# SDFIdk/malstroem

Hardware: NVIDIA B200
Metric: DEM cells/sec end-to-end (fill->D8->accum->bluespot/watershed labels) (higher is better)
Workload: dtype f32/f64

## Files before the change

malstroem_b200/csrc/common.cuh:

```cuda
#pragma once
#include <cuda_runtime.h>
#include <stdint.h>
#include <stdio.h>

#include "../../include/malstroem_b200.h"

namespace ms {

void set_error(const char *fmt, ...);
extern int64_t g_launches;

#define MS_CUDA(call)                                                                              \
    do {                                                                                           \
        cudaError_t e__ = (call);                                                                  \
        if (e__ != cudaSuccess) {                                                                  \
            ms::set_error("%s:%d: %s -> %s", __FILE__, __LINE__, #call, cudaGetErrorString(e__)); \
            return MS_ERR_CUDA;                                                                    \
        }                                                                                          \
    } while (0)

#define MS_TRY(call)                \
    do {                            \
        int r__ = (call);           \
        if (r__ != MS_OK) return r__; \
    } while (0)

extern int g_prof;
extern int64_t g_prof_units;
void prof_begin(const char *name, cudaStream_t s);
void prof_end(cudaStream_t s);
static inline void prof_units(int64_t u) { g_prof_units = u; }

#define MS_LAUNCH(kernel, grid, block, smem, stream, ...)                                    \
    do {                                                                                     \
        if (ms::g_prof) ms::prof_begin(#kernel, (stream));                                   \
        kernel<<<(grid), (block), (smem), (stream)>>>(__VA_ARGS__);                          \
        if (ms::g_prof) ms::prof_end((stream));                                              \
        ms::g_launches++;                                                                    \
        cudaError_t e__ = cudaGetLastError();                                                \
        if (e__ != cudaSuccess) {                                                            \
            ms::set_error("%s:%d: launch %s -> %s", __FILE__, __LINE__, #kernel,             \
                          cudaGetErrorString(e__));                                          \
            return MS_ERR_CUDA;                                                              \
        }                                                                                    \
    } while (0)

int ensure_init();

extern double g_host_t[4];
int stream_sync(cudaStream_t s);
double now_s();

void *arena_alloc(size_t bytes, cudaStream_t s);
void arena_free(void *p, cudaStream_t s);

template <typename T>
struct DevBuf {
    T *p = nullptr;
    cudaStream_t s = nullptr;
    DevBuf() {}
    DevBuf(const DevBuf &) = delete;
    DevBuf &operator=(const DevBuf &) = delete;
    int alloc(size_t n, cudaStream_t stream) {
        release();
        s = stream;
        if (n == 0) n = 1;
        double t0 = now_s();
        p = (T *)arena_alloc(n * sizeof(T), stream);
        g_host_t[2] += now_s() - t0;
        g_host_t[3] += 1;
        if (!p) {
            set_error("device scratch allocation of %zu bytes failed", n * sizeof(T));
            return MS_ERR_CUDA;
        }
        return MS_OK;
    }
    void release() {
        if (p) arena_free(p, s);
        p = nullptr;
    }
    ~DevBuf() { release(); }
    operator T *() const { return p; }
};

struct HostFlags {
    int64_t *h = nullptr;
    int init();
};
HostFlags &host_flags();
int readback(void *host_pinned, const void *dev, size_t bytes, cudaStream_t s);

static inline unsigned int cdiv(int64_t a, int64_t b) { return (unsigned int)((a + b - 1) / b); }

__host__ __device__ inline uint32_t okey32(float f) {
    f = f + 0.0f;
#ifdef __CUDA_ARCH__
    uint32_t b = __float_as_uint(f);
#else
    union { float f; uint32_t u; } v; v.f = f; uint32_t b = v.u;
#endif
    return (b & 0x80000000u) ? ~b : (b | 0x80000000u);
}
__host__ __device__ inline float okey32_inv(uint32_t k) {
    uint32_t b = (k & 0x80000000u) ? (k & 0x7fffffffu) : ~k;
#ifdef __CUDA_ARCH__
    return __uint_as_float(b);
#else
// ... 146 lines not shown
```

malstroem_b200/csrc/core.cu:

```cuda
#include <stdarg.h>
#include <stdio.h>
#include <stdlib.h>
#include <string.h>

#include <chrono>
#include <algorithm>
#include <map>
#include <string>
#include <vector>

#include "common.cuh"
#include "tma.cuh"

namespace ms {

static thread_local char g_err[1024] = "";
int64_t g_launches = 0;
static int g_device = -1;
static HostFlags g_flags;

void set_error(const char *fmt, ...) {
    va_list ap;
    va_start(ap, fmt);
    vsnprintf(g_err, sizeof(g_err), fmt, ap);
// ... 18 lines not shown

struct ArenaBlock { size_t off, size; bool live; };
static char *g_arena = nullptr;
static size_t g_arena_cap = 0, g_arena_top = 0, g_arena_need = 0, g_overflow_live = 0;
static std::vector<ArenaBlock> g_blocks;
static cudaStream_t g_arena_stream = nullptr;
static std::map<void *, size_t> g_overflow;

void *arena_alloc(size_t bytes, cudaStream_t s) {
    bytes = (bytes + 511) & ~(size_t)511;
    if (s != g_arena_stream) {
        if (g_arena) cudaStreamSynchronize(g_arena_stream);
        g_arena_stream = s;
    }
    if (g_blocks.empty() && g_overflow.empty() && g_arena_need > g_arena_cap) {
        if (g_arena) cudaFree(g_arena);
        g_arena = nullptr;
        size_t want = g_arena_need + (g_arena_need >> 3);
        if (cudaMalloc((void **)&g_arena, want) == cudaSuccess) g_arena_cap = want;
        else { g_arena_cap = 0; cudaGetLastError(); }
        g_arena_top = 0;
    }
    size_t virt = g_arena_top + g_overflow_live + bytes;
    if (virt > g_arena_need) g_arena_need = virt;
    if (g_arena && g_arena_top + bytes <= g_arena_cap) {
        g_blocks.push_back({g_arena_top, bytes, true});
        void *p = g_arena + g_arena_top;
        g_arena_top += bytes;
        return p;
    }
    void *p = nullptr;
    if (cudaMallocAsync(&p, bytes, s) != cudaSuccess) { cudaGetLastError(); return nullptr; }
    g_overflow[p] = bytes;
    g_overflow_live += bytes;
    return p;
}

void arena_free(void *p, cudaStream_t s) {
    auto it = g_overflow.find(p);
    if (it != g_overflow.end()) {
        g_overflow_live -= it->second;
        g_overflow.erase(it);
        cudaFreeAsync(p, s);
        return;
    }
    size_t off = (size_t)((char *)p - g_arena);
    for (size_t k = g_blocks.size(); k-- > 0;)
        if (g_blocks[k].off == off) { g_blocks[k].live = false; break; }
    while (!g_blocks.empty() && !g_blocks.back().live) {
        g_arena_top = g_blocks.back().off;
        g_blocks.pop_back();
    }
}

int g_prof = 0;
int64_t g_prof_units = 0;
struct ProfRec { const char *name; cudaEvent_t a, b; int64_t units; };
static std::vector<ProfRec> g_recs;
static std::vector<cudaEvent_t> g_evpool;

static cudaEvent_t ev_get() {
    if (!g_evpool.empty()) { cudaEvent_t e = g_evpool.back(); g_evpool.pop_back(); return e; }
    cudaEvent_t e;
    cudaEventCreate(&e);
    return e;
}

void prof_begin(const char *name, cudaStream_t s) {
    ProfRec r;
    r.name = name; r.a = ev_get(); r.b = ev_get(); r.units = g_prof_units;
    g_prof_units = 0;
    cudaEventRecord(r.a, s);
    g_recs.push_back(r);
}

void prof_end(cudaStream_t s) { cudaEventRecord(g_recs.back().b, s); }

int HostFlags::init() {
    if (h) return MS_OK;
    MS_CUDA(cudaHostAlloc((void **)&h, 64 * sizeof(int64_t), cudaHostAllocMapped | cudaHostAllocPortable));
    memset(h, 0, 64 * sizeof(int64_t));
    return MS_OK;
}
HostFlags &host_flags() { return g_flags; }

__global__ void k_readback(const uint32_t *__restrict__ src, uint32_t *dst_host, int words) {
    for (int k = threadIdx.x; k < words; k += blockDim.x) dst_host[k] = src[k];
    __threadfence_system();
}

int readback(void *host_pinned, const void *dev, size_t bytes, cudaStream_t s) {
    static int mode = -1;
    if (mode < 0) { const char *e = getenv("MS_READBACK"); mode = (e && e[0] == 'c') ? 0 : 1; }
    if (!mode || (bytes & 3) || bytes > 4096 || ((uintptr_t)dev & 3) || ((uintptr_t)host_pinned & 3)) {
        MS_CUDA(cudaMemcpyAsync(host_pinned, dev, bytes, cudaMemcpyDeviceToHost, s));
        return MS_OK;
    }
    MS_LAUNCH(k_readback, 1, 32, 0, s, (const uint32_t *)dev, (uint32_t *)host_pinned, (int)(bytes >> 2));
    return MS_OK;
}

static int init_device(int device) {
    int n = 0;
    cudaError_t e = cudaGetDeviceCount(&n);
    if (e != cudaSuccess || n == 0) {
        set_error("no CUDA device available (%s): malstroem_b200 has no CPU fallback",
// ... 274 lines not shown
```

malstroem_b200/csrc/fill.cu:

```cuda
#include <string.h>

#include "common.cuh"
#include "tma.cuh"

namespace ms {

constexpr unsigned long long KEY_NONE = ~0ull;

__global__ void __launch_bounds__(256) k_minmax(const float *z, int64_t n, uint32_t *keys, int vec) {
    uint32_t lo = 0xffffffffu, hi = 0u;
    int64_t i = ((int64_t)blockIdx.x * blockDim.x + threadIdx.x) * 4;
    int64_t stride = (int64_t)gridDim.x * blockDim.x * 4;
    for (; i < n; i += stride) {
        if (vec && i + 4 <= n) {
            float4 v = *reinterpret_cast<const float4 *>(z + i);
            uint32_t a = okey32(v.x), b = okey32(v.y), c = okey32(v.z), d = okey32(v.w);
            lo = min(lo, min(min(a, b), min(c, d)));
            hi = max(hi, max(max(a, b), max(c, d)));
        } else {
            for (int64_t j = i; j < n && j < i + 4; j++) {
                uint32_t a = okey32(z[j]);
                lo = min(lo, a);
                hi = max(hi, a);
            }
        }
    }
    lo = __reduce_min_sync(0xffffffffu, lo);
    hi = __reduce_max_sync(0xffffffffu, hi);
    __shared__ uint32_t slo[8], shi[8];
    int lane = threadIdx.x & 31, w = threadIdx.x >> 5;
    if (lane == 0) { slo[w] = lo; shi[w] = hi; }
    __syncthreads();
    if (w == 0) {
        lo = lane < 8 ? slo[lane] : 0xffffffffu;
        hi = lane < 8 ? shi[lane] : 0u;
        lo = __reduce_min_sync(0xffffffffu, lo);
        hi = __reduce_max_sync(0xffffffffu, hi);
        if (lane == 0) {
            atomicMin(&keys[0], lo);
            atomicMax(&keys[1], hi);
        }
    }
}

__global__ void k_minmax_finish(const uint32_t *keys, float *out) {
    out[0] = okey32_inv(keys[0]);
    out[1] = okey32_inv(keys[1]);
}

int minmax_dev(const float *z, int64_t n, float *out2, cudaStream_t s) {
    DevBuf<uint32_t> keys;
    MS_TRY(keys.alloc(2, s));
    static const uint32_t init[2] = {0xffffffffu, 0u};
    MS_CUDA(cudaMemcpyAsync(keys.p, init, sizeof(init), cudaMemcpyHostToDevice, s));
    int64_t want = (n / 4 + 255) / 256;
    int blocks = (int)(want < 1 ? 1 : (want > 148 * 16 ? 148 * 16 : want));
    MS_LAUNCH(k_minmax, blocks, 256, 0, s, z, n, keys.p, (int)(((uintptr_t)z & 15) == 0));
    MS_LAUNCH(k_minmax_finish, 1, 1, 0, s, keys.p, out2);
    return MS_OK;
}
// ... 49 lines not shown
                        if (r + dr < 0 || r + dr >= rows) continue;
                        int j = i + dr * cols + dc;
                        float zj = sz[(lr + 1 + dr) * LD + lc + X0 + dc];
                        if (zj < bz || (zj == bz && j < bi)) { bz = zj; bi = j; bdr = dr; bdc = dc; }
                    }
                int tr = lr + bdr, tc = lc + bdc;
                if (bi == i) t = i;
                else if (tr >= 0 && tr < FT && tc >= 0 && tc < FT) p = (unsigned short)(tr * FT + tc);
                else t = -(1 + bi);
            }
        }
        sp[k] = p;
        tgt[k] = t;
    }
    __syncthreads();
    tile_pointer_double(sp);
    int mine[16], cnt = 0;
#pragma unroll 4
    for (int u = 0; u < 16; u++) {
        int k = tid + 256 * u;
        int lr = k >> 6, lc = k & 63;
        int r = r0 + lr, c = c0 + lc;
        mine[u] = -1;
        if (r < rows && c < cols) {
            int t = tgt[sp[k]];
            int i = r * cols + c;
            if (t < 0) { t = -(t + 1); mine[u] = i; cnt++; }
            ptr[i] = t;
        }
    }
    int pos = block_append_pos(cnt, n_list);
#pragma unroll 4
    for (int u = 0; u < 16; u++)
        if (mine[u] >= 0) list[pos++] = mine[u];
}

__global__ void __launch_bounds__(256) k_catchment_ids(int *ptr_lab, const int *cid, int64_t n) {
    int64_t i = (int64_t)blockIdx.x * blockDim.x + threadIdx.x;
    if (i < n) ptr_lab[i] = cid[ptr_lab[i]];
}

__global__ void __launch_bounds__(256) k_boruvka_init(int *comp, uint32_t *E, int nC) {
    int l = blockIdx.x * blockDim.x + threadIdx.x;
    if (l < nC) {
        comp[l] = l;
        E[l] = okey32(-INFINITY);
    }
}

constexpr unsigned FOREIGN_BIT = 0x80000000u;

constexpr int ME_PER_THREAD = 4;

template <bool FIRST, bool BAND>
__device__ inline bool minedge_cell(const float *__restrict__ z, const int *__restrict__ lab,
                                    const int *__restrict__ comp, const uint8_t *__restrict__ frozen,
                                    unsigned long long *best, int rows, int cols, int i, int r, int c) {
    int l = lab[i];
    int cc = FIRST ? l : (l ? comp[l] : 0);
    if (cc == 0) return false;
    const bool fz = BAND && !FIRST && frozen[cc];
    bool other = false;
    float zc = z[i];
    unsigned long long bk = KEY_NONE;
#pragma unroll
    for (int dr = -1; dr <= 1; dr++)
#pragma unroll
        for (int dc = -1; dc <= 1; dc++) {
            if (dr == 0 && dc == 0) continue;
            int j = i + dr * cols + dc;
            if (r + dr < 0 || r + dr >= rows) {
                if (fz) { other = true; continue; }
                float w = fmaxf(zc, __ldg(z + j));
                if (c < 0) c = i % cols;
                unsigned long long key = ((unsigned long long)okey32(w) << 32) | FOREIGN_BIT | (unsigned)c;
                bk = key < bk ? key : bk;
                continue;
            }
            int lj = __ldg(lab + j);
            if (lj == l) continue;
            if (!FIRST && __ldg(comp + lj) == cc) continue;
            if (fz) { other = true; continue; }
            float w = fmaxf(zc, __ldg(z + j));
            int lo = j < i ? j : i;
            int code = (dr == 0) ? 0 : ((dr * dc == -1) ? 1 : (dc == 0 ? 2 : 3));
            unsigned long long key = ((unsigned long long)okey32(w) << 32) | (unsigned)(((unsigned)lo << 2) | code);
            bk = key < bk ? key : bk;
        }
    if (fz) return other;
    if (bk == KEY_NONE) return false;
    if (bk < best[cc]) atomicMin(&best[cc], bk);
    return true;
}

__device__ __forceinline__ void minedge_append(unsigned keepbits, const int (&cell)[ME_PER_THREAD], int *list_out, int *n_out) {
    __shared__ int wsum[8];
    __shared__ int base_s;
    int cnt = __popc(keepbits), lane = threadIdx.x & 31, w = threadIdx.x >> 5;
    int inc = cnt;
#pragma unroll
    for (int o = 1; o < 32; o <<= 1) {
        int y = __shfl_up_sync(0xffffffffu, inc, o);
        if (lane >= o) inc += y;
    }
    if (lane == 31) wsum[w] = inc;
    __syncthreads();
    if (threadIdx.x == 0) {
        int tot = 0;
        for (int k = 0; k < 8; k++) { int t = wsum[k]; wsum[k] = tot; tot += t; }
        base_s = tot ? atomicAdd(n_out, tot) : 0;
    }
    __syncthreads();
    int pos = base_s + wsum[w] + inc - cnt;
#pragma unroll
    for (int u = 0; u < ME_PER_THREAD; u++)
        if (keepbits & (1u << u)) list_out[pos++] = cell[u];
}

template <bool LIST, bool BAND>
__device__ __forceinline__ void minedge_body(const float *__restrict__ z, const int *__restrict__ lab,
                                                 const int *__restrict__ comp, const uint8_t *__restrict__ frozen,
                                                 unsigned long long *best, int rows, int cols,
                                                 const int *__restrict__ list_in, int n_in, int *list_out, int *n_out) {
    int cell[ME_PER_THREAD];
    unsigned keepbits = 0;
#pragma unroll
    for (int u = 0; u < ME_PER_THREAD; u++) {
        int i = -1, r = 0, c = 0;
        if (LIST) {
            int k = (blockIdx.x * ME_PER_THREAD + u) * 256 + threadIdx.x;
            if (k < n_in) {
                i = list_in[k];
                r = i < cols ? 0 : (i >= (rows - 1) * cols ? rows - 1 : 1);
                c = -1;
            }
        } else {
            c = blockIdx.x * 64 + (threadIdx.x & 63);
            r = (blockIdx.y * ME_PER_THREAD + u) * 4 + (threadIdx.x >> 6);
            if (r < rows && c < cols) i = r * cols + c;
        }
        cell[u] = i;
        if (i >= 0 && minedge_cell<!LIST, BAND>(z, lab, comp, frozen, best, rows, cols, i, r, c)) keepbits |= 1u << u;
    }
    minedge_append(keepbits, cell, list_out, n_out);
}

__global__ void __launch_bounds__(256) k_minedge_first4(const float *__restrict__ z, const int *__restrict__ lab,
                                                        unsigned long long *best, int rows, int cols, int *list_out,
                                                        int *n_out) {
    const int c = (blockIdx.x * 16 + (threadIdx.x & 15)) * 4;
    const int r = blockIdx.y * 16 + (threadIdx.x >> 4);
    int cell[ME_PER_THREAD] = {-1, -1, -1, -1};
    unsigned keepbits = 0;
    if (r > 0 && r < rows - 1 && c < cols) {
        int L[3][6];
        float Z[3][6];
#pragma unroll
        for (int a = 0; a < 3; a++) {
            const size_t row = (size_t)(r - 1 + a) * cols + c;
            const int4 l4 = __ldg(reinterpret_cast<const int4 *>(lab + row));
            const float4 z4 = __ldg(reinterpret_cast<const float4 *>(z + row));
            L[a][1] = l4.x; L[a][2] = l4.y; L[a][3] = l4.z; L[a][4] = l4.w;
            Z[a][1] = z4.x; Z[a][2] = z4.y; Z[a][3] = z4.z; Z[a][4] = z4.w;
            L[a][0] = c > 0 ? __ldg(lab + row - 1) : 0;
            Z[a][0] = c > 0 ? __ldg(z + row - 1) : 0.f;
            L[a][5] = c + 4 < cols ? __ldg(lab + row + 4) : 0;
            Z[a][5] = c + 4 < cols ? __ldg(z + row + 4) : 0.f;
        }
#pragma unroll
        for (int j = 0; j < 4; j++) {
            const int l = L[1][j + 1];
            const int i = r * cols + c + j;
            cell[j] = i;
            if (l == 0) continue;
            const float zc = Z[1][j + 1];
            unsigned long long bk = KEY_NONE;
#pragma unroll
            for (int dr = -1; dr <= 1; dr++)
#pragma unroll
                for (int dc = -1; dc <= 1; dc++) {
                    if (dr == 0 && dc == 0) continue;
                    if (L[1 + dr][j + 1 + dc] == l) continue;
                    const float w = fmaxf(zc, Z[1 + dr][j + 1 + dc]);
                    const int jn = i + dr * cols + dc;
                    const int lo = jn < i ? jn : i;
                    const int code = (dr == 0) ? 0 : ((dr * dc == -1) ? 1 : (dc == 0 ? 2 : 3));
                    const unsigned long long key = ((unsigned long long)okey32(w) << 32) | (unsigned)(((unsigned)lo << 2) | code);
                    bk = key < bk ? key : bk;
                }
            if (bk == KEY_NONE) continue;
            if (bk < best[l]) atomicMin(&best[l], bk);
            keepbits |= 1u << j;
        }
    }
    minedge_append(keepbits, cell, list_out, n_out);
}

template <bool LIST>
__global__ void __launch_bounds__(256) k_minedge(const float *__restrict__ z, const int *__restrict__ lab,
                                                 const int *__restrict__ comp, const uint8_t *__restrict__ frozen,
                                                 unsigned long long *best, int rows, int cols,
                                                 const int *__restrict__ list_in, int n_in, int *list_out, int *n_out) {
    minedge_body<LIST, false>(z, lab, comp, frozen, best, rows, cols, list_in, n_in, list_out, n_out);
}
template <bool LIST>
__global__ void __launch_bounds__(256) k_minedge_band(const float *__restrict__ z, const int *__restrict__ lab,
                                                      const int *__restrict__ comp, const uint8_t *__restrict__ frozen,
                                                      unsigned long long *best, int rows, int cols,
                                                      const int *__restrict__ list_in, int n_in, int *list_out, int *n_out) {
    minedge_body<LIST, true>(z, lab, comp, frozen, best, rows, cols, list_in, n_in, list_out, n_out);
}

__device__ inline int edge_other(int lo, int code, int cols) {
    return lo + (code == 0 ? 1 : (code == 1 ? cols - 1 : (code == 2 ? cols : cols + 1)));
}

__global__ void __launch_bounds__(256) k_hook(const unsigned long long *__restrict__ best,
                                              const int *__restrict__ comp, const int *__restrict__ lab,
                                              int *parent, uint32_t *wk, uint8_t *frozen, int nC, int cols) {
    int k = blockIdx.x * blockDim.x + threadIdx.x;
    if (k >= nC) return;
    parent[k] = k;
    wk[k] = okey32(-INFINITY);
    if (k == 0 || comp[k] != k) return;
    unsigned long long b = best[k];
    if (b == KEY_NONE) return;
    unsigned id = (unsigned)(b & 0xffffffffu);
    if (frozen && (id & FOREIGN_BIT)) {
        frozen[k] = 1;
        return;
    }
    int lo = (int)(id >> 2), code = (int)(id & 3u);
    int hi = edge_other(lo, code, cols);
    int ca = comp[lab[lo]], cb = comp[lab[hi]];
    int t = (ca == k) ? cb : ca;
    wk[k] = (uint32_t)(b >> 32);
    if (t != 0 && best[t] == b && k < t) t = k;
    parent[k] = t;
}

__device__ inline int uf_find(int *parent, int k) {
    int p = parent[k];
    for (;;) {
        int g = parent[p];
        if (g == p) return p;
        parent[k] = g;
        k = p;
        p = g;
    }
}

__global__ void __launch_bounds__(256) k_boruvka_update(int *comp, uint32_t *E, int *parent,
                                                        const uint32_t *__restrict__ wk,
                                                        const uint8_t *__restrict__ frozen, int nC,
                                                        unsigned long long *best, int *remaining) {
    int l = blockIdx.x * blockDim.x + threadIdx.x;
    int live = 0;
    if (l < nC) {
        best[l] = KEY_NONE;
        int k = comp[l];
        if (k != 0) {
            uint32_t e = E[l], w = wk[k];
            if (w > e) E[l] = w;
            int r = uf_find(parent, k);
            comp[l] = r;
            live = (r == l) && !(frozen && frozen[r]);
        }
    }
    int cnt = __syncthreads_count(live);
    if (threadIdx.x == 0 && cnt) atomicAdd(remaining, cnt);
}

__global__ void __launch_bounds__(256) k_fill_final(const float *__restrict__ z, const int *__restrict__ lab,
                                                    const uint32_t *__restrict__ E, float *__restrict__ filled,
                                                    float *__restrict__ depths, int64_t n) {
    int64_t i = (int64_t)blockIdx.x * blockDim.x + threadIdx.x;
    if (i >= n) return;
    float zc = z[i];
    float w = fmaxf(zc, okey32_inv(__ldg(E + lab[i])));
    filled[i] = w;
    if (depths) depths[i] = __fsub_rn(w, zc);
}

static int descent_resolve(const float *dem, int *lab, int *scratch, int64_t rows, int64_t cols, int open,
                           int64_t *rounds_out, cudaStream_t s) {
    DevBuf<int> cnt;
    MS_TRY(cnt.alloc(1, s));
    MS_CUDA(cudaMemsetAsync(cnt.p, 0, sizeof(int), s));
    int tiles_x = (int)cdiv(cols, FT), tiles_y = (int)cdiv(rows, FT);
    prof_units(rows * cols);
    CUtensorMap zmap;
    memset(&zmap, 0, sizeof(zmap));
    if (!open && tma_map_2d(&zmap, dem, rows, cols, FT + 2, DT_LD_TMA, true, true))
        MS_LAUNCH(k_descent_tile<true>, tiles_x * tiles_y, 256, 0, s, dem, lab, (int)rows, (int)cols, tiles_x, open, scratch, cnt.p, zmap);
    else
        MS_LAUNCH(k_descent_tile<false>, tiles_x * tiles_y, 256, 0, s, dem, lab, (int)rows, (int)cols, tiles_x, open, scratch, cnt.p, zmap);
    int64_t *h = host_flags().h;
    MS_TRY(ms::readback(h, cnt.p, sizeof(int), s));
    MS_TRY(ms::stream_sync(s));
    return forest_resolve_list(lab, scratch, *(int *)h, rounds_out, s);
}

static int boruvka_rounds(const float *dem, const int *lab, int *comp, uint32_t *E, uint8_t *frozen, int nC,
                          int64_t rows, int64_t cols, int *rounds_out, const char *what, cudaStream_t s,
                          ms_band *B = nullptr) {
    int64_t n = rows * cols;
    DevBuf<int> parent, counters, listA, listB;
    DevBuf<uint32_t> wk;
    DevBuf<unsigned long long> best;
    MS_TRY(parent.alloc(nC, s));
    MS_TRY(wk.alloc(nC, s));
    MS_TRY(best.alloc(nC, s));
    MS_TRY(counters.alloc(2, s));
    MS_TRY(listA.alloc((size_t)n, s));
    dim3 g2(cdiv(cols, 64), cdiv(rows, 4));
    unsigned gc = cdiv(nC, 256);
    int64_t *h = host_flags().h;
    MS_CUDA(cudaMemsetAsync(best.p, 0xff, (size_t)nC * sizeof(unsigned long long), s));
    int rounds = 0;
    int64_t live = nC - 1;
    int n_list = 0;
    int *lin = nullptr, *lout = listA.p;
    while (live > 0) {
        MS_CUDA(cudaMemsetAsync(counters.p, 0, 2 * sizeof(int), s));
        if (rounds == 0) {
            prof_units(n);
            dim3 g2m(cdiv(cols, 64), cdiv(rows, 4 * ME_PER_THREAD));
            if (frozen)
                MS_LAUNCH(k_minedge_band<false>, g2m, 256, 0, s, dem, lab, (const int *)comp, (const uint8_t *)frozen, best.p,
                          (int)rows, (int)cols, (const int *)nullptr, 0, lout, counters.p + 1);
            else if ((cols & 3) == 0 && ((uintptr_t)dem & 15) == 0 && ((uintptr_t)lab & 15) == 0)
                MS_LAUNCH(k_minedge_first4, dim3(cdiv(cols, 64), cdiv(rows, 16)), 256, 0, s, dem, lab, best.p, (int)rows, (int)cols,
                          lout, counters.p + 1);
            else
                MS_LAUNCH(k_minedge<false>, g2m, 256, 0, s, dem, lab, (const int *)comp, (const uint8_t *)frozen, best.p,
                          (int)rows, (int)cols, (const int *)nullptr, 0, lout, counters.p + 1);
        } else {
            prof_units(n_list);
            if (frozen)
                MS_LAUNCH(k_minedge_band<true>, cdiv(n_list, 256 * ME_PER_THREAD), 256, 0, s, dem, lab, (const int *)comp,
                          (const uint8_t *)frozen, best.p, (int)rows, (int)cols, (const int *)lin, n_list, lout, counters.p + 1);
            else
                MS_LAUNCH(k_minedge<true>, cdiv(n_list, 256 * ME_PER_THREAD), 256, 0, s, dem, lab, (const int *)comp,
                          (const uint8_t *)frozen, best.p, (int)rows, (int)cols, (const int *)lin, n_list, lout, counters.p + 1);
        }
        MS_LAUNCH(k_hook, gc, 256, 0, s, best.p, comp, lab, parent.p, wk.p, frozen, nC, (int)cols);
        MS_LAUNCH(k_boruvka_update, gc, 256, 0, s, comp, E, parent.p, wk.p, (const uint8_t *)frozen, nC, best.p,
                  counters.p);
        MS_TRY(ms::readback(h, counters.p, 2 * sizeof(int), s));
        MS_TRY(ms::stream_sync(s));
        int64_t now = ((int *)h)[0];
        n_list = ((int *)h)[1];
        rounds++;
        if (now >= live || rounds > 64) {
            set_error("%s: Boruvka contraction stalled (%lld -> %lld live components, round %d)", what,
                      (long long)live, (long long)now, rounds);
            return MS_ERR_NOCONV;
        }
        live = now;
        if (live > 0 && n_list == 0) {
            set_error("%s: live components without an outgoing edge", what);
            return MS_ERR_NOCONV;
        }
        if (rounds == 1 && live > 0) MS_TRY(listB.alloc((size_t)n_list, s));
        lin = lout;
        lout = (lout == listA.p) ? listB.p : listA.p;
    }
    if (rounds_out) *rounds_out = rounds;
    if (B) {
        B->n_blist = 0;
        if (rounds > 0 && n_list > 0) {
            int *dst = (int *)band_buf(B, BB_BLIST, (size_t)n_list * sizeof(int));
            if (!dst) return MS_ERR_CUDA;
            MS_CUDA(cudaMemcpyAsync(dst, lin, (size_t)n_list * sizeof(int), cudaMemcpyDeviceToDevice, s));
            MS_TRY(ms::stream_sync(s));
            B->n_blist = n_list;
        }
    }
    return MS_OK;
}

int fill_terrain_dev_impl(const float *dtm, float *filled, float *depths, int64_t rows, int64_t cols,
                          int64_t *stats, cudaStream_t s) {
    if (!dtm || !filled) { set_error("fill_terrain: null pointer"); return MS_ERR_ARG; }
    if (rows < 3 || cols < 3 || rows * cols > (1ll << 30)) {
        set_error("fill_terrain: unsupported shape %lld x %lld", (long long)rows, (long long)cols);
        return MS_ERR_SHAPE;
    }
    int64_t n = rows * cols;
    DevBuf<int> lab, tmp;
    DevBuf<int64_t> total;
    MS_TRY(lab.alloc((size_t)n, s));
    MS_TRY(tmp.alloc((size_t)n, s));
    MS_TRY(total.alloc(1, s));
    dim3 g2(cdiv(cols, 64), cdiv(rows, 4));
    unsigned g1 = cdiv(n, 256);
    int64_t *h = host_flags().h;

    int64_t jump_rounds = 0;
    MS_TRY(descent_resolve(dtm, lab.p, tmp.p, rows, cols, 0, &jump_rounds, s));
    MS_TRY(exclusive_scan_selfptr(lab.p, tmp.p, n, total.p, s));
    MS_LAUNCH(k_catchment_ids, g1, 256, 0, s, lab.p, tmp.p, n);
    MS_TRY(ms::readback(h, total.p, sizeof(int64_t), s));
    MS_TRY(ms::stream_sync(s));
    int nC = (int)h[0];
    tmp.release();

    DevBuf<int> comp;
    DevBuf<uint32_t> E;
    MS_TRY(comp.alloc(nC, s));
    MS_TRY(E.alloc(nC, s));
    MS_LAUNCH(k_boruvka_init, cdiv(nC, 256), 256, 0, s, comp.p, E.p, nC);
    int rounds = 0;
    MS_TRY(boruvka_rounds(dtm, lab.p, comp.p, E.p, nullptr, nC, rows, cols, &rounds, "fill_terrain", s));
    MS_LAUNCH(k_fill_final, g1, 256, 0, s, dtm, lab.p, E.p, filled, depths, n);
    if (stats) { stats[0] = rounds; stats[1] = nC; stats[5] = jump_rounds; }
    return MS_OK;
}


__global__ void __launch_bounds__(256) k_frozen_flags(const int *comp, const uint8_t *frozen, int *flag, int nC) {
    int k = blockIdx.x * blockDim.x + threadIdx.x;
    if (k < nC) flag[k] = (k != 0 && comp[k] == k && frozen[k]) ? 1 : 0;
}

__device__ inline int band_gid(int K, const int *frank, int base) { return K ? 1 + base + frank[K] : 0; }

__global__ void __launch_bounds__(256) k_band_edge_ids(const int *__restrict__ lab, const int *__restrict__ comp,
                                                       const int *__restrict__ frank, int base, int rows, int cols,
                                                       int32_t *top, int32_t *bot) {
    int c = blockIdx.x * blockDim.x + threadIdx.x;
    if (c >= cols) return;
    top[c] = band_gid(comp[lab[c]], frank, base);
    bot[c] = band_gid(comp[lab[(size_t)(rows - 1) * cols + c]], frank, base);
}

constexpr unsigned long long HASH_EMPTY = ~0ull;

__device__ inline void edge_insert(unsigned long long *hk, uint32_t *hv, unsigned H, int ga, int gb, uint32_t w,
                                   int *overflow) {
    int a = ga < gb ? ga : gb, b = ga < gb ? gb : ga;
    unsigned long long key = ((unsigned long long)(unsigned)a << 32) | (unsigned)b;
    unsigned long long x = key * 0x9E3779B97F4A7C15ull;
    unsigned h = (unsigned)(x >> 32) & (H - 1);
    for (unsigned probes = 0; probes < H; probes++) {
        unsigned long long cur = hk[h];
        if (cur == HASH_EMPTY) {
            unsigned long long old = atomicCAS(hk + h, HASH_EMPTY, key);
            cur = (old == HASH_EMPTY) ? key : old;
        }
        if (cur == key) {
            if (w < hv[h]) atomicMin(hv + h, w);
            return;
        }
        h = (h + 1) & (H - 1);
    }
    *overflow = 1;
}

__global__ void __launch_bounds__(256) k_band_edges(const float *__restrict__ z, const int *__restrict__ lab,
                                                    const int *__restrict__ comp, const int *__restrict__ frank,
                                                    int base, const int32_t *__restrict__ halo_top,
                                                    const int32_t *__restrict__ halo_bot, int rows, int cols,
                                                    unsigned long long *hk, uint32_t *hv, unsigned H, int *overflow,
                                                    const int *__restrict__ list, int n_list) {
    int k = blockIdx.x * blockDim.x + threadIdx.x;
    if (k >= n_list) return;
    int i = list[k];
    int r = i / cols, c = i - r * cols;
    int l = lab[i];
    if (l == 0) return;
    int K = comp[l];
    if (K == 0) return;
    int ga = band_gid(K, frank, base);
    float zc = z[i];
    int last_gb = -1;
    uint32_t last_w = 0;
#pragma unroll
    for (int dr = -1; dr <= 1; dr++)
#pragma unroll
        for (int dc = -1; dc <= 1; dc++) {
            if (dr == 0 && dc == 0) continue;
            int j = i + dr * cols + dc;
            int gb;
            if (r + dr < 0) gb = halo_top[c + dc];
            else if (r + dr >= rows) gb = halo_bot[c + dc];
            else {
                int lj = __ldg(lab + j);
                if (lj == l) continue;
                int Kj = lj ? __ldg(comp + lj) : 0;
// ... 33 lines not shown
        int changed = 0;
        for (int e = threadIdx.x; e < ne; e += blockDim.x) {
            int a = ea[e], b = eb[e];
            uint32_t w = okey32(ew[e]);
            uint32_t xa = *(volatile uint32_t *)(X + a), xb = *(volatile uint32_t *)(X + b);
            uint32_t ca = w > xb ? w : xb, cb = w > xa ? w : xa;
            if (ca < xa) { atomicMin(X + a, ca); changed = 1; }
            if (cb < xb) { atomicMin(X + b, cb); changed = 1; }
        }
        if (!__syncthreads_or(changed)) break;
    }
    for (int k = threadIdx.x; k < nn; k += blockDim.x) out[k] = okey32_inv(X[k]);
    if (threadIdx.x == 0 && iters) *iters = it;
}

__global__ void __launch_bounds__(256) k_band_raise(uint32_t *E, const int *__restrict__ comp,
                                                    const int *__restrict__ frank, int base,
                                                    const float *__restrict__ X, int nC) {
    int l = blockIdx.x * blockDim.x + threadIdx.x;
    if (l >= nC || l == 0) return;
    int K = comp[l];
    if (K == 0) return;
    uint32_t x = okey32(X[band_gid(K, frank, base)]);
    if (x > E[l]) E[l] = x;
}

int fill_band_local(ms_band *B, const float *dem, int64_t *n_frozen, cudaStream_t s) {
    int64_t rows = B->rows, cols = B->cols, n = rows * cols;
    int *lab = (int *)band_buf(B, BB_LAB, (size_t)n * sizeof(int));
    if (!lab) return MS_ERR_CUDA;
    DevBuf<int> tmp;
    DevBuf<int64_t> total;
    MS_TRY(tmp.alloc((size_t)n, s));
    MS_TRY(total.alloc(1, s));
    dim3 g2(cdiv(cols, 64), cdiv(rows, 4));
    unsigned g1 = cdiv(n, 256);
    int64_t *h = host_flags().h;
    MS_TRY(descent_resolve(dem, lab, tmp.p, rows, cols, B->open, nullptr, s));
    MS_TRY(exclusive_scan_selfptr(lab, tmp.p, n, total.p, s));
    MS_LAUNCH(k_catchment_ids, g1, 256, 0, s, lab, tmp.p, n);
    MS_TRY(ms::readback(h, total.p, sizeof(int64_t), s));
    MS_TRY(ms::stream_sync(s));
    int nC = (int)h[0];
    tmp.release();
    B->nC = nC;
    int *comp = (int *)band_buf(B, BB_COMP, (size_t)nC * sizeof(int));
    uint32_t *E = (uint32_t *)band_buf(B, BB_E, (size_t)nC * sizeof(uint32_t));
    uint8_t *frozen = (uint8_t *)band_buf(B, BB_FROZEN, (size_t)nC);
    int *frank = (int *)band_buf(B, BB_FRANK, (size_t)nC * sizeof(int));
    if (!comp || !E || !frozen || !frank) return MS_ERR_CUDA;
    unsigned gc = cdiv(nC, 256);
    MS_LAUNCH(k_boruvka_init, gc, 256, 0, s, comp, E, nC);
    MS_CUDA(cudaMemsetAsync(frozen, 0, (size_t)nC, s));
    MS_TRY(boruvka_rounds(dem, lab, comp, E, frozen, nC, rows, cols, nullptr, "band fill", s, B));
    MS_LAUNCH(k_frozen_flags, gc, 256, 0, s, comp, frozen, frank, nC);
    MS_TRY(exclusive_scan_i32(frank, frank, nC, total.p, s));
    MS_TRY(ms::readback(h, total.p, sizeof(int64_t), s));
    MS_TRY(ms::stream_sync(s));
    B->nF = (int)h[0];
    if (n_frozen) *n_frozen = B->nF;
    return MS_OK;
}

}

extern "C" {

int ms_band_fill_local_dev(ms_band *B, const float *dem, int64_t *n_frozen, void *stream) {
    MS_TRY(ms::ensure_init());
    if (!B || !dem) { ms::set_error("band fill: null pointer"); return MS_ERR_ARG; }
    return ms::fill_band_local(B, dem, n_frozen, (cudaStream_t)stream);
}

int ms_band_fill_edge_ids_dev(ms_band *B, int64_t gid_base, int32_t *gid_top, int32_t *gid_bot, void *stream) {
    using namespace ms;
    MS_TRY(ensure_init());
    if (!B || !gid_top || !gid_bot || !B->buf[BB_LAB]) { set_error("band fill: edge ids before the local phase"); return MS_ERR_ARG; }
    cudaStream_t s = (cudaStream_t)stream;
    B->gid_base = (int)gid_base;
    MS_LAUNCH(k_band_edge_ids, cdiv(B->cols, 256), 256, 0, s, (const int *)B->buf[BB_LAB], (const int *)B->buf[BB_COMP],
              (const int *)B->buf[BB_FRANK], B->gid_base, (int)B->rows, (int)B->cols, gid_top, gid_bot);
    return MS_OK;
}

int ms_band_fill_edges_dev(ms_band *B, const float *dem, const int32_t *halo_gid_top, const int32_t *halo_gid_bot,
                           int32_t *edge_a, int32_t *edge_b, float *edge_w, int64_t capacity, int64_t *n_edges,
                           void *stream) {
    using namespace ms;
    MS_TRY(ensure_init());
    if (!B || !dem || !edge_a || !edge_b || !edge_w || !n_edges) { set_error("band fill: null pointer"); return MS_ERR_ARG; }
    if (((B->open & 1) && !halo_gid_top) || ((B->open & 2) && !halo_gid_bot)) {
        set_error("band fill: halo component ids missing for an open band edge");
        return MS_ERR_ARG;
    }
    cudaStream_t s = (cudaStream_t)stream;
    int64_t *h = host_flags().h;
    unsigned H = 4096;
    while ((int64_t)H < 16ll * ((int64_t)B->nF + B->cols)) H <<= 1;
    for (int attempt = 0; attempt < 6; attempt++, H <<= 1) {
        unsigned long long *hk = (unsigned long long *)band_buf(B, BB_HASHK, (size_t)H * 8);
        uint32_t *hv = (uint32_t *)band_buf(B, BB_HASHV, (size_t)H * 4);
        int *cnt = (int *)band_buf(B, BB_MISC, 64);
        if (!hk || !hv || !cnt) return MS_ERR_CUDA;
        MS_CUDA(cudaMemsetAsync(hk, 0xff, (size_t)H * 8, s));
        MS_CUDA(cudaMemsetAsync(hv, 0xff, (size_t)H * 4, s));
        MS_CUDA(cudaMemsetAsync(cnt, 0, 64, s));
        if (B->n_blist > 0)
// ... 112 lines not shown
```

Measured before the change: 5975.

## Replace per-cell Boruvka fill with tile-built catchment edge list contraction

```diff
diff --git a/malstroem_b200/csrc/common.cuh b/malstroem_b200/csrc/common.cuh
--- a/malstroem_b200/csrc/common.cuh
+++ b/malstroem_b200/csrc/common.cuh
@@ -53,6 +53,7 @@
 
 void *arena_alloc(size_t bytes, cudaStream_t s);
 void arena_free(void *p, cudaStream_t s);
+size_t arena_room();
 
 template <typename T>
 struct DevBuf {
diff --git a/malstroem_b200/csrc/core.cu b/malstroem_b200/csrc/core.cu
--- a/malstroem_b200/csrc/core.cu
+++ b/malstroem_b200/csrc/core.cu
@@ -94,6 +94,8 @@
         g_blocks.pop_back();
     }
 }
+
+size_t arena_room() { return g_arena ? g_arena_cap - g_arena_top : 0; }
 
 int g_prof = 0;
 int64_t g_prof_units = 0;
diff --git a/malstroem_b200/csrc/fill.cu b/malstroem_b200/csrc/fill.cu
--- a/malstroem_b200/csrc/fill.cu
+++ b/malstroem_b200/csrc/fill.cu
@@ -6,6 +6,7 @@
 namespace ms {
 
 constexpr unsigned long long KEY_NONE = ~0ull;
+constexpr unsigned long long HASH_EMPTY = ~0ull;
 
 __global__ void __launch_bounds__(256) k_minmax(const float *z, int64_t n, uint32_t *keys, int vec) {
     uint32_t lo = 0xffffffffu, hi = 0u;
@@ -161,14 +162,14 @@
 
 constexpr int ME_PER_THREAD = 4;
 
-template <bool FIRST, bool BAND>
+template <bool FIRST>
 __device__ inline bool minedge_cell(const float *__restrict__ z, const int *__restrict__ lab,
                                     const int *__restrict__ comp, const uint8_t *__restrict__ frozen,
                                     unsigned long long *best, int rows, int cols, int i, int r, int c) {
     int l = lab[i];
     int cc = FIRST ? l : (l ? comp[l] : 0);
     if (cc == 0) return false;
-    const bool fz = BAND && !FIRST && frozen[cc];
+    const bool fz = !FIRST && frozen[cc];
     bool other = false;
     float zc = z[i];
     unsigned long long bk = KEY_NONE;
@@ -226,11 +227,11 @@
         if (keepbits & (1u << u)) list_out[pos++] = cell[u];
 }
 
-template <bool LIST, bool BAND>
-__device__ __forceinline__ void minedge_body(const float *__restrict__ z, const int *__restrict__ lab,
-                                                 const int *__restrict__ comp, const uint8_t *__restrict__ frozen,
-                                                 unsigned long long *best, int rows, int cols,
-                                                 const int *__restrict__ list_in, int n_in, int *list_out, int *n_out) {
+template <bool LIST>
+__global__ void __launch_bounds__(256) k_minedge_band(const float *__restrict__ z, const int *__restrict__ lab,
+                                                      const int *__restrict__ comp, const uint8_t *__restrict__ frozen,
+                                                      unsigned long long *best, int rows, int cols,
+                                                      const int *__restrict__ list_in, int n_in, int *list_out, int *n_out) {
     int cell[ME_PER_THREAD];
     unsigned keepbits = 0;
 #pragma unroll
@@ -249,75 +250,9 @@
             if (r < rows && c < cols) i = r * cols + c;
         }
         cell[u] = i;
-        if (i >= 0 && minedge_cell<!LIST, BAND>(z, lab, comp, frozen, best, rows, cols, i, r, c)) keepbits |= 1u << u;
+        if (i >= 0 && minedge_cell<!LIST>(z, lab, comp, frozen, best, rows, cols, i, r, c)) keepbits |= 1u << u;
     }
     minedge_append(keepbits, cell, list_out, n_out);
-}
-
-__global__ void __launch_bounds__(256) k_minedge_first4(const float *__restrict__ z, const int *__restrict__ lab,
-                                                        unsigned long long *best, int rows, int cols, int *list_out,
-                                                        int *n_out) {
-    const int c = (blockIdx.x * 16 + (threadIdx.x & 15)) * 4;
-    const int r = blockIdx.y * 16 + (threadIdx.x >> 4);
-    int cell[ME_PER_THREAD] = {-1, -1, -1, -1};
-    unsigned keepbits = 0;
-    if (r > 0 && r < rows - 1 && c < cols) {
-        int L[3][6];
-        float Z[3][6];
-#pragma unroll
-        for (int a = 0; a < 3; a++) {
-            const size_t row = (size_t)(r - 1 + a) * cols + c;
-            const int4 l4 = __ldg(reinterpret_cast<const int4 *>(lab + row));
-            const float4 z4 = __ldg(reinterpret_cast<const float4 *>(z + row));
-            L[a][1] = l4.x; L[a][2] = l4.y; L[a][3] = l4.z; L[a][4] = l4.w;
-            Z[a][1] = z4.x; Z[a][2] = z4.y; Z[a][3] = z4.z; Z[a][4] = z4.w;
-            L[a][0] = c > 0 ? __ldg(lab + row - 1) : 0;
-            Z[a][0] = c > 0 ? __ldg(z + row - 1) : 0.f;
-            L[a][5] = c + 4 < cols ? __ldg(lab + row + 4) : 0;
-            Z[a][5] = c + 4 < cols ? __ldg(z + row + 4) : 0.f;
-        }
-#pragma unroll
-        for (int j = 0; j < 4; j++) {
-            const int l = L[1][j + 1];
-            const int i = r * cols + c + j;
-            cell[j] = i;
-            if (l == 0) continue;
-            const float zc = Z[1][j + 1];
-            unsigned long long bk = KEY_NONE;
-#pragma unroll
-            for (int dr = -1; dr <= 1; dr++)
-#pragma unroll
-                for (int dc = -1; dc <= 1; dc++) {
-                    if (dr == 0 && dc == 0) continue;
-                    if (L[1 + dr][j + 1 + dc] == l) continue;
-                    const float w = fmaxf(zc, Z[1 + dr][j + 1 + dc]);
-                    const int jn = i + dr * cols + dc;
-                    const int lo = jn < i ? jn : i;
-                    const int code = (dr == 0) ? 0 : ((dr * dc == -1) ? 1 : (dc == 0 ? 2 : 3));
-                    const unsigned long long key = ((unsigned long long)okey32(w) << 32) | (unsigned)(((unsigned)lo << 2) | code);
-                    bk = key < bk ? key : bk;
-                }
-            if (bk == KEY_NONE) continue;
-            if (bk < best[l]) atomicMin(&best[l], bk);
-            keepbits |= 1u << j;
-        }
-    }
-    minedge_append(keepbits, cell, list_out, n_out);
-}
-
-template <bool LIST>
-__global__ void __launch_bounds__(256) k_minedge(const float *__restrict__ z, const int *__restrict__ lab,
-                                                 const int *__restrict__ comp, const uint8_t *__restrict__ frozen,
-                                                 unsigned long long *best, int rows, int cols,
-                                                 const int *__restrict__ list_in, int n_in, int *list_out, int *n_out) {
-    minedge_body<LIST, false>(z, lab, comp, frozen, best, rows, cols, list_in, n_in, list_out, n_out);
-}
-template <bool LIST>
-__global__ void __launch_bounds__(256) k_minedge_band(const float *__restrict__ z, const int *__restrict__ lab,
-                                                      const int *__restrict__ comp, const uint8_t *__restrict__ frozen,
-                                                      unsigned long long *best, int rows, int cols,
-                                                      const int *__restrict__ list_in, int n_in, int *list_out, int *n_out) {
-    minedge_body<LIST, true>(z, lab, comp, frozen, best, rows, cols, list_in, n_in, list_out, n_out);
 }
 
 __device__ inline int edge_other(int lo, int code, int cols) {
@@ -410,9 +345,8 @@
     return forest_resolve_list(lab, scratch, *(int *)h, rounds_out, s);
 }
 
-static int boruvka_rounds(const float *dem, const int *lab, int *comp, uint32_t *E, uint8_t *frozen, int nC,
-                          int64_t rows, int64_t cols, int *rounds_out, const char *what, cudaStream_t s,
-                          ms_band *B = nullptr) {
+static int boruvka_rounds_band(const float *dem, const int *lab, int *comp, uint32_t *E, uint8_t *frozen, int nC,
+                               int64_t rows, int64_t cols, cudaStream_t s, ms_band *B) {
     int64_t n = rows * cols;
     DevBuf<int> parent, counters, listA, listB;
     DevBuf<uint32_t> wk;
@@ -422,7 +356,6 @@
     MS_TRY(best.alloc(nC, s));
     MS_TRY(counters.alloc(2, s));
     MS_TRY(listA.alloc((size_t)n, s));
-    dim3 g2(cdiv(cols, 64), cdiv(rows, 4));
     unsigned gc = cdiv(nC, 256);
     int64_t *h = host_flags().h;
     MS_CUDA(cudaMemsetAsync(best.p, 0xff, (size_t)nC * sizeof(unsigned long long), s));
@@ -435,23 +368,12 @@
         if (rounds == 0) {
             prof_units(n);
             dim3 g2m(cdiv(cols, 64), cdiv(rows, 4 * ME_PER_THREAD));
-            if (frozen)
-                MS_LAUNCH(k_minedge_band<false>, g2m, 256, 0, s, dem, lab, (const int *)comp, (const uint8_t *)frozen, best.p,
-                          (int)rows, (int)cols, (const int *)nullptr, 0, lout, counters.p + 1);
-            else if ((cols & 3) == 0 && ((uintptr_t)dem & 15) == 0 && ((uintptr_t)lab & 15) == 0)
-                MS_LAUNCH(k_minedge_first4, dim3(cdiv(cols, 64), cdiv(rows, 16)), 256, 0, s, dem, lab, best.p, (int)rows, (int)cols,
-                          lout, counters.p + 1);
-            else
-                MS_LAUNCH(k_minedge<false>, g2m, 256, 0, s, dem, lab, (const int *)comp, (const uint8_t *)frozen, best.p,
-                          (int)rows, (int)cols, (const int *)nullptr, 0, lout, counters.p + 1);
+            MS_LAUNCH(k_minedge_band<false>, g2m, 256, 0, s, dem, lab, (const int *)comp, (const uint8_t *)frozen, best.p,
+                      (int)rows, (int)cols, (const int *)nullptr, 0, lout, counters.p + 1);
         } else {
             prof_units(n_list);
-            if (frozen)
-                MS_LAUNCH(k_minedge_band<true>, cdiv(n_list, 256 * ME_PER_THREAD), 256, 0, s, dem, lab, (const int *)comp,
-                          (const uint8_t *)frozen, best.p, (int)rows, (int)cols, (const int *)lin, n_list, lout, counters.p + 1);
-            else
-                MS_LAUNCH(k_minedge<true>, cdiv(n_list, 256 * ME_PER_THREAD), 256, 0, s, dem, lab, (const int *)comp,
-                          (const uint8_t *)frozen, best.p, (int)rows, (int)cols, (const int *)lin, n_list, lout, counters.p + 1);
+            MS_LAUNCH(k_minedge_band<true>, cdiv(n_list, 256 * ME_PER_THREAD), 256, 0, s, dem, lab, (const int *)comp,
+                      (const uint8_t *)frozen, best.p, (int)rows, (int)cols, (const int *)lin, n_list, lout, counters.p + 1);
         }
         MS_LAUNCH(k_hook, gc, 256, 0, s, best.p, comp, lab, parent.p, wk.p, frozen, nC, (int)cols);
         MS_LAUNCH(k_boruvka_update, gc, 256, 0, s, comp, E, parent.p, wk.p, (const uint8_t *)frozen, nC, best.p,
@@ -462,31 +384,207 @@
         n_list = ((int *)h)[1];
         rounds++;
         if (now >= live || rounds > 64) {
-            set_error("%s: Boruvka contraction stalled (%lld -> %lld live components, round %d)", what,
+            set_error("band fill: Boruvka contraction stalled (%lld -> %lld live components, round %d)",
                       (long long)live, (long long)now, rounds);
             return MS_ERR_NOCONV;
         }
         live = now;
         if (live > 0 && n_list == 0) {
-            set_error("%s: live components without an outgoing edge", what);
+            set_error("band fill: live components without an outgoing edge");
             return MS_ERR_NOCONV;
         }
         if (rounds == 1 && live > 0) MS_TRY(listB.alloc((size_t)n_list, s));
         lin = lout;
         lout = (lout == listA.p) ? listB.p : listA.p;
     }
-    if (rounds_out) *rounds_out = rounds;
-    if (B) {
-        B->n_blist = 0;
-        if (rounds > 0 && n_list > 0) {
-            int *dst = (int *)band_buf(B, BB_BLIST, (size_t)n_list * sizeof(int));
-            if (!dst) return MS_ERR_CUDA;
-            MS_CUDA(cudaMemcpyAsync(dst, lin, (size_t)n_list * sizeof(int), cudaMemcpyDeviceToDevice, s));
-            MS_TRY(ms::stream_sync(s));
-            B->n_blist = n_list;
-        }
+    B->n_blist = 0;
+    if (rounds > 0 && n_list > 0) {
+        int *dst = (int *)band_buf(B, BB_BLIST, (size_t)n_list * sizeof(int));
+        if (!dst) return MS_ERR_CUDA;
+        MS_CUDA(cudaMemcpyAsync(dst, lin, (size_t)n_list * sizeof(int), cudaMemcpyDeviceToDevice, s));
+        MS_TRY(ms::stream_sync(s));
+        B->n_blist = n_list;
     }
     return MS_OK;
+}
+
+constexpr int TE_SLOTS = 1024;
+constexpr int TE_PROBES = 32;
+constexpr int TE_LD = FT + 2;
+constexpr int TE_N = (FT + 1) * TE_LD;
+constexpr int TE_LOADS = (TE_N + 255) / 256;
+
+__device__ __forceinline__ void edge_put(int *ea, int *eb, uint32_t *ew, unsigned long long *best, int pos, int a, int b,
+                                         uint32_t w) {
+    ea[pos] = a;
+    eb[pos] = b;
+    ew[pos] = w;
+    unsigned long long key = ((unsigned long long)w << 32) | (unsigned)pos;
+    if (a && key < best[a]) atomicMin(&best[a], key);
+    if (key < best[b]) atomicMin(&best[b], key);
+}
+
+__device__ __forceinline__ void tile_edge_insert(unsigned long long *hk, uint32_t *hw, int a, int b, uint32_t w,
+                                                 int *ea, int *eb, uint32_t *ew, int cap, int *n_edges,
+                                                 unsigned long long *best) {
+    unsigned long long key = ((unsigned long long)(unsigned)a << 32) | (unsigned)b;
+    unsigned h = (unsigned)((key * 0x9E3779B97F4A7C15ull) >> 32) & (TE_SLOTS - 1);
+    for (int p = 0; p < TE_PROBES; p++) {
+        unsigned long long cur = hk[h];
+        if (cur == HASH_EMPTY) {
+            unsigned long long old = atomicCAS(hk + h, HASH_EMPTY, key);
+            cur = (old == HASH_EMPTY) ? key : old;
+        }
+        if (cur == key) {
+            atomicMin(hw + h, w);
+            return;
+        }
+        h = (h + 1) & (TE_SLOTS - 1);
+    }
+    int pos = atomicAdd(n_edges, 1);
+    if (pos < cap) edge_put(ea, eb, ew, best, pos, a, b, w);
+}
+
+template <bool TMA>
+__global__ void __launch_bounds__(256) k_tile_edges(const float *__restrict__ z, const int *__restrict__ ptr,
+                                                    const int *__restrict__ cid, int *__restrict__ lab, int rows,
+                                                    int cols, int tiles_x, int *ea, int *eb, uint32_t *ew, int cap,
+                                                    int *n_edges, unsigned long long *best,
+                                                    const __grid_constant__ CUtensorMap zmap) {
+    constexpr int LD = TMA ? DT_LD_TMA : FT + 2;
+    constexpr int X0 = TMA ? DT_X0_TMA : 1;
+    __shared__ __align__(128) float sz[(FT + 2) * LD];
+    __shared__ int sl[TE_N];
+    __shared__ unsigned long long hk[TE_SLOTS];
+    __shared__ uint32_t hw[TE_SLOTS];
+    __shared__ uint64_t bar;
+    int ty = blockIdx.x / tiles_x, tx = blockIdx.x - ty * tiles_x;
+    int r0 = ty * FT, c0 = tx * FT, tid = threadIdx.x;
+    for (int k = tid; k < TE_SLOTS; k += 256) { hk[k] = HASH_EMPTY; hw[k] = 0xffffffffu; }
+    if (TMA) {
+        if (tid == 0) mbar_init(&bar, 1);
+        __syncthreads();
+        if (tid == 0) {
+            mbar_expect_tx(&bar, (unsigned)sizeof(sz));
+            tma_load_2d(sz, &zmap, &bar, c0 - DT_X0_TMA, r0 - 1);
+        }
+    } else {
+        for (int k = tid; k < (FT + 2) * (FT + 2); k += 256) {
+            int lr = k / (FT + 2), lc = k - lr * (FT + 2);
+            int r = r0 + lr - 1, c = c0 + lc - 1;
+            sz[k] = (r >= 0 && r < rows && c >= 0 && c < cols) ? z[(size_t)r * cols + c] : INFINITY;
+        }
+    }
+    int pv[TE_LOADS];
+#pragma unroll
+    for (int u = 0; u < TE_LOADS; u++) {
+        int k = tid + 256 * u, lr = k / TE_LD, lc = k - lr * TE_LD;
+        int r = r0 + lr, c = c0 + lc - 1;
+        pv[u] = (k < TE_N && r < rows && c >= 0 && c < cols) ? __ldg(ptr + (size_t)r * cols + c) : -1;
+    }
+#pragma unroll
+    for (int u = 0; u < TE_LOADS; u++) {
+        int k = tid + 256 * u, lr = k / TE_LD, lc = k - lr * TE_LD;
+        if (k >= TE_N) break;
+        int l = pv[u] >= 0 ? __ldg(cid + pv[u]) : -1;
+        sl[k] = l;
+        if (l >= 0 && lr < FT && lc >= 1 && lc <= FT) lab[(size_t)(r0 + lr) * cols + c0 + lc - 1] = l;
+    }
+    if (TMA) mbar_wait(&bar, 0);
+    __syncthreads();
+    const int lc = tid & 63, lr0 = (tid >> 6) * 16, c = c0 + lc;
+    int pa = -1, pb = -1;
+    uint32_t pw = 0;
+    if (c < cols) {
+        for (int u = 0; u < 16; u++) {
+            const int lr = lr0 + u, r = r0 + lr;
+            if (r >= rows) break;
+            const int l = sl[lr * TE_LD + lc + 1];
+            const float zc = sz[(lr + 1) * LD + lc + X0];
+#pragma unroll
+            for (int d = 0; d < 4; d++) {
+                const int dr = d == 0 ? 0 : 1, dc = d == 0 ? 1 : d - 2;
+                if (r + dr >= rows || c + dc < 0 || c + dc >= cols) continue;
+                const int m = sl[(lr + dr) * TE_LD + lc + 1 + dc];
+                if (m == l) continue;
+                const uint32_t w = okey32(fmaxf(zc, sz[(lr + 1 + dr) * LD + lc + X0 + dc]));
+                const int a = min(l, m), b = max(l, m);
+                if (a == pa && b == pb) { pw = min(pw, w); continue; }
+                if (pa >= 0) tile_edge_insert(hk, hw, pa, pb, pw, ea, eb, ew, cap, n_edges, best);
+                pa = a; pb = b; pw = w;
+            }
+        }
+    }
+    if (pa >= 0) tile_edge_insert(hk, hw, pa, pb, pw, ea, eb, ew, cap, n_edges, best);
+    __syncthreads();
+    int cnt = 0;
+#pragma unroll
+    for (int k = tid; k < TE_SLOTS; k += 256) cnt += hk[k] != HASH_EMPTY;
+    int pos = block_append_pos(cnt, n_edges);
+#pragma unroll
+    for (int k = tid; k < TE_SLOTS; k += 256) {
+        unsigned long long key = hk[k];
+        if (key == HASH_EMPTY) continue;
+        if (pos < cap) edge_put(ea, eb, ew, best, pos, (int)(key >> 32), (int)(key & 0xffffffffu), hw[k]);
+        pos++;
+    }
+}
+
+__global__ void __launch_bounds__(256) k_hook_edges(const unsigned long long *__restrict__ best,
+                                                    const int *__restrict__ ea, const int *__restrict__ eb,
+                                                    int *parent, uint32_t *wk, int *flag, int V) {
+    int v = blockIdx.x * blockDim.x + threadIdx.x;
+    if (v >= V) return;
+    int p = v;
+    uint32_t w = okey32(-INFINITY);
+    unsigned long long b = v ? best[v] : KEY_NONE;
+    if (b != KEY_NONE) {
+        unsigned e = (unsigned)(b & 0xffffffffu);
+        int x = ea[e], y = eb[e];
+        int t = (x == v) ? y : x;
+        w = (uint32_t)(b >> 32);
+        if (t != 0 && best[t] == b && v < t) t = v;
+        p = t;
+    }
+    parent[v] = p;
+    wk[v] = w;
+    flag[v] = (v != 0 && p == v) ? 1 : 0;
+}
+
+__global__ void __launch_bounds__(256) k_level_map(int *parent, const int *__restrict__ nid, int *map, int V) {
+    int v = blockIdx.x * blockDim.x + threadIdx.x;
+    if (v >= V) return;
+    int r = uf_find(parent, v);
+    map[v] = r ? nid[r] + 1 : 0;
+}
+
+__global__ void __launch_bounds__(256) k_edges_relabel(const int *__restrict__ ia, const int *__restrict__ ib,
+                                                       const uint32_t *__restrict__ iw, int m,
+                                                       const int *__restrict__ map, int *oa, int *ob, uint32_t *ow,
+                                                       int *n_out, unsigned long long *best) {
+    int e = blockIdx.x * blockDim.x + threadIdx.x;
+    int a = 0, b = 0;
+    uint32_t w = 0;
+    if (e < m) {
+        a = __ldg(map + ia[e]);
+        b = __ldg(map + ib[e]);
+        w = iw[e];
+        if (a > b) { int t = a; a = b; b = t; }
+    }
+    int keep = a != b;
+    int pos = block_append_pos(keep, n_out);
+    if (keep) edge_put(oa, ob, ow, best, pos, a, b, w);
+}
+
+__global__ void __launch_bounds__(256) k_spill_down(uint32_t *wk, const int *__restrict__ map,
+                                                    const uint32_t *__restrict__ x_up, int V) {
+    int v = blockIdx.x * blockDim.x + threadIdx.x;
+    if (v >= V) return;
+    int u = map[v];
+    if (u) {
+        uint32_t x = x_up[u];
+        if (x > wk[v]) wk[v] = x;
+    }
 }
 
 int fill_terrain_dev_impl(const float *dtm, float *filled, float *depths, int64_t rows, int64_t cols,
@@ -497,32 +595,117 @@
         return MS_ERR_SHAPE;
     }
     int64_t n = rows * cols;
-    DevBuf<int> lab, tmp;
-    DevBuf<int64_t> total;
+    DevBuf<int> lab, ptr, cid;
+    DevBuf<int64_t> ctr;
     MS_TRY(lab.alloc((size_t)n, s));
-    MS_TRY(tmp.alloc((size_t)n, s));
-    MS_TRY(total.alloc(1, s));
-    dim3 g2(cdiv(cols, 64), cdiv(rows, 4));
-    unsigned g1 = cdiv(n, 256);
+    MS_TRY(ptr.alloc((size_t)n, s));
+    MS_TRY(cid.alloc((size_t)n, s));
+    MS_TRY(ctr.alloc(2, s));
     int64_t *h = host_flags().h;
 
     int64_t jump_rounds = 0;
-    MS_TRY(descent_resolve(dtm, lab.p, tmp.p, rows, cols, 0, &jump_rounds, s));
-    MS_TRY(exclusive_scan_selfptr(lab.p, tmp.p, n, total.p, s));
-    MS_LAUNCH(k_catchment_ids, g1, 256, 0, s, lab.p, tmp.p, n);
-    MS_TRY(ms::readback(h, total.p, sizeof(int64_t), s));
+    MS_TRY(descent_resolve(dtm, ptr.p, cid.p, rows, cols, 0, &jump_rounds, s));
+    MS_TRY(exclusive_scan_selfptr(ptr.p, cid.p, n, ctr.p, s));
+    MS_TRY(ms::readback(h, ctr.p, sizeof(int64_t), s));
     MS_TRY(ms::stream_sync(s));
-    int nC = (int)h[0];
-    tmp.release();
-
-    DevBuf<int> comp;
-    DevBuf<uint32_t> E;
-    MS_TRY(comp.alloc(nC, s));
-    MS_TRY(E.alloc(nC, s));
-    MS_LAUNCH(k_boruvka_init, cdiv(nC, 256), 256, 0, s, comp.p, E.p, nC);
-    int rounds = 0;
-    MS_TRY(boruvka_rounds(dtm, lab.p, comp.p, E.p, nullptr, nC, rows, cols, &rounds, "fill_terrain", s));
-    MS_LAUNCH(k_fill_final, g1, 256, 0, s, dtm, lab.p, E.p, filled, depths, n);
+    const int nC = (int)h[0];
+
+    const int64_t lv_cap = 2 * (int64_t)nC + 64;
+    DevBuf<unsigned long long> best;
+    DevBuf<int> parent, nid, map_all;
+    DevBuf<uint32_t> wk_all;
+    MS_TRY(best.alloc(nC, s));
+    MS_TRY(parent.alloc(nC, s));
+    MS_TRY(nid.alloc(nC, s));
+    MS_TRY(map_all.alloc((size_t)lv_cap, s));
+    MS_TRY(wk_all.alloc((size_t)lv_cap, s));
+
+    const int64_t cap_max = n * 4 < 0x7fffffffll ? n * 4 : 0x7fffffffll;
+    int64_t cap = (int64_t)(arena_room() / (2 * (2 * sizeof(int) + sizeof(uint32_t))));
+    if (cap < n / 16 + 4096) cap = n / 16 + 4096;
+    if (cap > cap_max) cap = cap_max;
+    DevBuf<int> ea[2], eb[2];
+    DevBuf<uint32_t> ew[2];
+    CUtensorMap zmap;
+    memset(&zmap, 0, sizeof(zmap));
+    const bool tma = tma_map_2d(&zmap, dtm, rows, cols, FT + 2, DT_LD_TMA, true, true);
+    const int tiles_x = (int)cdiv(cols, FT), tiles = tiles_x * (int)cdiv(rows, FT);
+    int64_t m = 0;
+    for (int attempt = 0;; attempt++) {
+        MS_TRY(ea[0].alloc((size_t)cap, s));
+        MS_TRY(eb[0].alloc((size_t)cap, s));
+        MS_TRY(ew[0].alloc((size_t)cap, s));
+        MS_CUDA(cudaMemsetAsync(best.p, 0xff, (size_t)nC * sizeof(unsigned long long), s));
+        MS_CUDA(cudaMemsetAsync(ctr.p + 1, 0, sizeof(int64_t), s));
+        prof_units(n);
+        if (tma)
+            MS_LAUNCH(k_tile_edges<true>, tiles, 256, 0, s, dtm, ptr.p, cid.p, lab.p, (int)rows, (int)cols, tiles_x, ea[0].p,
+                      eb[0].p, ew[0].p, (int)cap, (int *)(ctr.p + 1), best.p, zmap);
+        else
+            MS_LAUNCH(k_tile_edges<false>, tiles, 256, 0, s, dtm, ptr.p, cid.p, lab.p, (int)rows, (int)cols, tiles_x, ea[0].p,
+                      eb[0].p, ew[0].p, (int)cap, (int *)(ctr.p + 1), best.p, zmap);
+        MS_TRY(ms::readback(h, ctr.p + 1, sizeof(int), s));
+        MS_TRY(ms::stream_sync(s));
+        m = (int64_t)(unsigned)((int *)h)[0];
+        if (m <= cap) break;
+        if (attempt > 0 || cap == cap_max) {
+            set_error("fill_terrain: %lld catchment edges do not fit the list (%lld)", (long long)m, (long long)cap);
+            return MS_ERR_NOCONV;
+        }
+        ew[0].release();
+        eb[0].release();
+        ea[0].release();
+        cap = m + m / 4 < cap_max ? m + m / 4 : cap_max;
+    }
+    cid.release();
+    ptr.release();
+    MS_TRY(ea[1].alloc((size_t)m, s));
+    MS_TRY(eb[1].alloc((size_t)m, s));
+    MS_TRY(ew[1].alloc((size_t)m, s));
+
+    int64_t lv_off[66];
+    int64_t V = nC, live = nC - 1;
+    int rounds = 0, cur = 0;
+    lv_off[0] = 0;
+    if (live == 0) MS_LAUNCH(k_hook_edges, 1, 256, 0, s, best.p, ea[0].p, eb[0].p, parent.p, wk_all.p, nid.p, (int)V);
+    while (live > 0) {
+        uint32_t *wk = wk_all.p + lv_off[rounds];
+        int *map = map_all.p + lv_off[rounds];
+        unsigned gv = cdiv(V, 256);
+        MS_LAUNCH(k_hook_edges, gv, 256, 0, s, best.p, ea[cur].p, eb[cur].p, parent.p, wk, nid.p, (int)V);
+        MS_TRY(exclusive_scan_i32(nid.p, nid.p, V, ctr.p, s));
+        MS_LAUNCH(k_level_map, gv, 256, 0, s, parent.p, nid.p, map, (int)V);
+        MS_CUDA(cudaMemsetAsync(best.p, 0xff, (size_t)V * sizeof(unsigned long long), s));
+        MS_CUDA(cudaMemsetAsync(ctr.p + 1, 0, sizeof(int64_t), s));
+        prof_units(m);
+        if (m > 0)
+            MS_LAUNCH(k_edges_relabel, cdiv(m, 256), 256, 0, s, ea[cur].p, eb[cur].p, ew[cur].p, (int)m, map, ea[1 - cur].p,
+                      eb[1 - cur].p, ew[1 - cur].p, (int *)(ctr.p + 1), best.p);
+        MS_TRY(ms::readback(h, ctr.p, 2 * sizeof(int64_t), s));
+        MS_TRY(ms::stream_sync(s));
+        int64_t now = h[0];
+        m = (int64_t)((int *)(h + 1))[0];
+        rounds++;
+        lv_off[rounds] = lv_off[rounds - 1] + V;
+        if (now >= live || rounds > 64 || lv_off[rounds] + now + 1 > lv_cap) {
+            set_error("fill_terrain: Boruvka contraction stalled (%lld -> %lld live components, round %d)",
+                      (long long)live, (long long)now, rounds);
+            return MS_ERR_NOCONV;
+        }
+        live = now;
+        if (live > 0 && m == 0) {
+            set_error("fill_terrain: live components without an outgoing edge");
+            return MS_ERR_NOCONV;
+        }
+        V = live + 1;
+        cur = 1 - cur;
+    }
+    for (int t = rounds - 2; t >= 0; t--) {
+        int64_t Vt = lv_off[t + 1] - lv_off[t];
+        MS_LAUNCH(k_spill_down, cdiv(Vt, 256), 256, 0, s, wk_all.p + lv_off[t], (const int *)map_all.p + lv_off[t],
+                  (const uint32_t *)wk_all.p + lv_off[t + 1], (int)Vt);
+    }
+    MS_LAUNCH(k_fill_final, cdiv(n, 256), 256, 0, s, dtm, lab.p, wk_all.p, filled, depths, n);
     if (stats) { stats[0] = rounds; stats[1] = nC; stats[5] = jump_rounds; }
     return MS_OK;
 }
@@ -543,8 +726,6 @@
     top[c] = band_gid(comp[lab[c]], frank, base);
     bot[c] = band_gid(comp[lab[(size_t)(rows - 1) * cols + c]], frank, base);
 }
-
-constexpr unsigned long long HASH_EMPTY = ~0ull;
 
 __device__ inline void edge_insert(unsigned long long *hk, uint32_t *hv, unsigned H, int ga, int gb, uint32_t w,
                                    int *overflow) {
@@ -684,7 +865,7 @@
     unsigned gc = cdiv(nC, 256);
     MS_LAUNCH(k_boruvka_init, gc, 256, 0, s, comp, E, nC);
     MS_CUDA(cudaMemsetAsync(frozen, 0, (size_t)nC, s));
-    MS_TRY(boruvka_rounds(dem, lab, comp, E, frozen, nC, rows, cols, nullptr, "band fill", s, B));
+    MS_TRY(boruvka_rounds_band(dem, lab, comp, E, frozen, nC, rows, cols, s, B));
     MS_LAUNCH(k_frozen_flags, gc, 256, 0, s, comp, frozen, frank, nC);
     MS_TRY(exclusive_scan_i32(frank, frank, nC, total.p, s));
     MS_TRY(ms::readback(h, total.p, sizeof(int64_t), s));
```

Measured after the change: 6763 (median of 6 runs). 13.2% higher.
